# KevynUtopia/Frequency-Aware-Inverse-Consistent-OCTA-Super-Resolution

Measured on AMD Instinct MI355X. Metric: train-step images/sec (G+D fwd+bwd) on 256x256 OCTA, higher is better.
Workload: dtype f32 (tensors and accumulators fp32; the convolutions' operands enter the matrix cores as f16x2 pairs: hi = f16(x 2^k), lo = f16(x 2^k - hi), k from the tensor's largest magnitude; 3 v_mfma_f32_32x32x16_f16 per product) on every map >= 24 wide with >= 16 channels; narrow maps, 1-channel stems / head

## Files before the change

### frequency-aware-inverse-consistent-octa-super-resolution_amd/csrc/common.h

```cpp
#pragma once
#include <hip/hip_runtime.h>
#include <cstdio>
#include <cstdarg>
#include "faoctasr.h"

namespace faoctasr {

char* err_buf();
int fail(int code, const char* fmt, ...);
enum Route { ROUTE_NONE = 0, ROUTE_GATHER_FLAT = 1, ROUTE_PATCH = 2, ROUTE_WINOGRAD = 3, ROUTE_BF16X3 = 4, ROUTE_M1_FWD = 5, ROUTE_NARROW = 6,
             ROUTE_WGRAD_FLAT = 11, ROUTE_WGRAD_PATCH = 12, ROUTE_WGRAD_S1 = 13, ROUTE_M1_WGRAD = 14, ROUTE_WGRAD_X3 = 15, ROUTE_STEM_DGRAD = 7, ROUTE_STEM_WGRAD = 16,
             ROUTE_NARROW_X2 = 8 };
void set_route(int r);
extern thread_local int g_no_split_k;
extern thread_local unsigned* g_out_absmax;
unsigned* take_out_absmax();

void lds_optin(const void* kernel, size_t lds_bytes);

inline int check_launch(const char* what) {
    hipError_t e = hipGetLastError();
    if (e != hipSuccess) return fail(FAOCTASR_EHIP, "%s: %s", what, hipGetErrorString(e));
    return FAOCTASR_OK;
}

__device__ __forceinline__ float act_apply(float v, int act, float slope) {
    switch (act) {
        case FAOCTASR_ACT_RELU: return v > 0.f ? v : 0.f;
        case FAOCTASR_ACT_LRELU: return v > 0.f ? v : v * slope;
        case FAOCTASR_ACT_TANH: return tanhf(v);
        default: return v;
    }
}
__device__ __forceinline__ float act_grad_from_out(float y, int act, float slope) {
    switch (act) {
        case FAOCTASR_ACT_RELU: return y > 0.f ? 1.f : 0.f;
        case FAOCTASR_ACT_LRELU: return y > 0.f ? 1.f : slope;
        case FAOCTASR_ACT_TANH: return 1.f - y * y;
        default: return 1.f;
    }
}

template <class T>
__device__ __forceinline__ T wave_sum(T v) {
#pragma unroll
    for (int o = 32; o > 0; o >>= 1) v += __shfl_xor(v, o, 64);
    return v;
}

template <class T>
__device__ __forceinline__ T block_sum_256(T v, T* red ) {
    v = wave_sum(v);
    __syncthreads();
    if ((threadIdx.x & 63) == 0) red[threadIdx.x >> 6] = v;
    __syncthreads();
    return red[0] + red[1] + red[2] + red[3];
}

__device__ __forceinline__ void block_partial_store_256(float v, float* red , float* part) {
    v = block_sum_256(v, red);
    if (threadIdx.x == 0) part[blockIdx.x] = v;
}

template <class T>
__device__ __forceinline__ double strided_sum_256(const T* __restrict__ p, long n) {
    double a = 0.0;
    for (long i = threadIdx.x; i < n; i += 256) a += (double)p[i];
    return a;
}

__device__ __forceinline__ double block_tree_256(double v, double* red ) {
    red[threadIdx.x] = v;
    __syncthreads();
    for (int o = 128; o > 0; o >>= 1) {
        if ((int)threadIdx.x < o) red[threadIdx.x] += red[threadIdx.x + o];
        __syncthreads();
    }
    const double s = red[0];
    __syncthreads();
    return s;
}

struct PlaneTile { int plane, y0, x0; };
template <int TY, int TX>
__device__ __forceinline__ PlaneTile plane_tile(int tiles_h, int tiles_w) {
    unsigned bi = blockIdx.x;
    PlaneTile t;
    t.x0 = (int)(bi % (unsigned)tiles_w) * TX; bi /= (unsigned)tiles_w;
    t.y0 = (int)(bi % (unsigned)tiles_h) * TY;
    t.plane = (int)(bi / (unsigned)tiles_h);
    return t;
}

inline bool plane_tiles(long planes, int h, int w, int TY, int TX, int* tiles_h, int* tiles_w, long* blocks) {
    *tiles_h = (h + TY - 1) / TY;
    *tiles_w = (w + TX - 1) / TX;
    const long per_plane = (long)*tiles_h * *tiles_w;
    if (planes > 0x7fffffffL / per_plane) return false;
    *blocks = planes * per_plane;
    return true;
}

}
```

### frequency-aware-inverse-consistent-octa-super-resolution_amd/csrc/conv_m1.hip

```cpp
#include "common.h"

namespace faoctasr {

constexpr int M1_TH = 8, M1_TW = 32, M1_KC = 16;

__global__ __launch_bounds__(256) void conv_m1_fwd_kernel(const float* __restrict__ x, const float* __restrict__ w,
                                                          const float* __restrict__ bias, float* __restrict__ y, int N, int C,
                                                          int H, int W, int KH, int KW, int pad, int act, float slope) {
    extern __shared__ __attribute__((aligned(16))) char smem[];
    float* P = reinterpret_cast<float*>(smem);
    const int PH = M1_TH + KH - 1, PW = M1_TW + KW - 1, PHW = PH * PW, T = KH * KW;
    float* Wl = P + M1_KC * PHW;
    const int tid = threadIdx.x;
    const int tiles_x = (W + M1_TW - 1) / M1_TW, tiles_y = (H + M1_TH - 1) / M1_TH;
    const int n = blockIdx.x / (tiles_x * tiles_y);
    const int r = blockIdx.x - n * tiles_x * tiles_y;
    const int y0 = (r / tiles_x) * M1_TH, x0 = (r % tiles_x) * M1_TW;
    const int ty = tid >> 5, tx = tid & 31;
    const long hw = (long)H * W;
    const float* xn = x + (long)n * C * hw;
    constexpr unsigned OOB = 0x7fffffffu;
    const float invPHW = 1.0f / (float)PHW, invPW = 1.0f / (float)PW;
    float acc = 0.f;
    for (int c0 = 0; c0 < C; c0 += M1_KC) {
        const long bytes = (long)(C - c0) * hw * 4;
        const auto srd = __builtin_amdgcn_make_buffer_rsrc(const_cast<float*>(xn + (long)c0 * hw), 0,
                                                           (int)(bytes < 0x7ffffff0L ? bytes : 0x7ffffff0L), 0x00020000);
        __syncthreads();
        for (int e = tid; e < M1_KC * PHW; e += 256) {
            const int c = (int)(((float)e + 0.5f) * invPHW);
            const int q = e - c * PHW;
            const int py = (int)(((float)q + 0.5f) * invPW);
            const int iy = y0 - pad + py, ix = x0 - pad + (q - py * PW);
            const bool ok = (unsigned)iy < (unsigned)H && (unsigned)ix < (unsigned)W;
            P[e] = __builtin_bit_cast(float, __builtin_amdgcn_raw_buffer_load_b32(srd, ok ? 4u * (unsigned)(c * (int)hw + iy * W + ix) : OOB, 0, 0));
        }
        for (int e = tid; e < M1_KC * T; e += 256) Wl[e] = (c0 + e / T < C) ? w[(long)c0 * T + e] : 0.f;
        __syncthreads();
        const float* pp = P + ty * PW + tx;
        for (int c = 0; c < M1_KC; ++c)
            for (int kh = 0; kh < KH; ++kh)
                for (int kw = 0; kw < KW; ++kw) acc += Wl[c * T + kh * KW + kw] * pp[c * PHW + kh * PW + kw];
    }
    const int oy = y0 + ty, ox = x0 + tx;
    if (oy < H && ox < W) {
        if (bias) acc += bias[0];
        y[(long)n * hw + (long)oy * W + ox] = act_apply(acc, act, slope);
    }
}

__global__ __launch_bounds__(256) void conv_m1_wgrad_kernel(const float* __restrict__ x, const float* __restrict__ dy,
                                                            float* __restrict__ dw, int N, int C, int H, int W, int KH, int KW, int pad,
                                                            int tiles_per_block, int CCH) {
    extern __shared__ __attribute__((aligned(16))) char smem[];
    const int PH = M1_TH + KH - 1, PW = M1_TW + KW - 1, PHW = PH * PW, T = KH * KW;
    float* P = reinterpret_cast<float*>(smem);
    float* D = P + CCH * PHW;
    const int tid = threadIdx.x;
    const int c0 = blockIdx.y * CCH;
    const int cl = tid / T, t = tid - cl * T;
    const bool mine = cl < CCH && c0 + cl < C;
    const int kh = t / KW, kw = t - kh * KW;
    const int tiles_x = (W + M1_TW - 1) / M1_TW, tiles_y = (H + M1_TH - 1) / M1_TH;
    const long ntiles = (long)N * tiles_x * tiles_y;
    const long hw = (long)H * W;
    constexpr unsigned OOB = 0x7fffffffu;
    const float invPHW = 1.0f / (float)PHW, invPW = 1.0f / (float)PW;
    float acc = 0.f;
    long tile = (long)blockIdx.x * tiles_per_block;
    long tend = tile + tiles_per_block;
    tend = tend < ntiles ? tend : ntiles;
    for (; tile < tend; ++tile) {
        const int n = (int)(tile / (tiles_x * tiles_y));
        const int r = (int)(tile - (long)n * tiles_x * tiles_y);
        const int y0 = (r / tiles_x) * M1_TH, x0 = (r % tiles_x) * M1_TW;
        const long bytes = (long)(C - c0) * hw * 4;
        const auto srd = __builtin_amdgcn_make_buffer_rsrc(const_cast<float*>(x + ((long)n * C + c0) * hw), 0,
                                                           (int)(bytes < 0x7ffffff0L ? bytes : 0x7ffffff0L), 0x00020000);
        __syncthreads();
        for (int e = tid; e < CCH * PHW; e += 256) {
            const int c = (int)(((float)e + 0.5f) * invPHW);
            const int q = e - c * PHW;
            const int py = (int)(((float)q + 0.5f) * invPW);
            const int iy = y0 - pad + py, ix = x0 - pad + (q - py * PW);
            const bool ok = (unsigned)iy < (unsigned)H && (unsigned)ix < (unsigned)W;
            P[e] = __builtin_bit_cast(float, __builtin_amdgcn_raw_buffer_load_b32(srd, ok ? 4u * (unsigned)(c * (int)hw + iy * W + ix) : OOB, 0, 0));
        }
        {
            const int py = tid >> 5, px = tid & 31;
            const int oy = y0 + py, ox = x0 + px;
            D[tid] = (oy < H && ox < W) ? dy[(long)n * hw + (long)oy * W + ox] : 0.f;
        }
        __syncthreads();
        if (mine) {
            const float* pp = P + cl * PHW + kh * PW + kw;
#pragma unroll 4
            for (int py = 0; py < M1_TH; ++py)
#pragma unroll 8
                for (int px = 0; px < M1_TW; ++px) acc += D[py * M1_TW + px] * pp[py * PW + px];
        }
    }
    if (mine) atomicAdd(dw + (long)(c0 + cl) * T + t, acc);
}

typedef float m1f4 __attribute__((ext_vector_type(4)));

__device__ __forceinline__ void m1_row6(const float* __restrict__ row, int xq, int W, bool rowok, float (&v)[6]) {
    m1f4 c = {0.f, 0.f, 0.f, 0.f};
    float l = 0.f, r = 0.f;
    if (rowok) {
        c = *reinterpret_cast<const m1f4*>(row + xq);
        if (xq > 0) l = row[xq - 1];
        if (xq + 4 < W) r = row[xq + 4];
    }
    v[0] = l; v[1] = c[0]; v[2] = c[1]; v[3] = c[2]; v[4] = c[3]; v[5] = r;
}

__global__ __launch_bounds__(256) void conv_m1_fwd3_kernel(const float* __restrict__ x, const float* __restrict__ w, const float* __restrict__ bias,
                                                           float* __restrict__ y, int N, int C, int H, int W, int act, float slope) {
    const int wq = W >> 2;
    const long item = (long)blockIdx.x * 256 + threadIdx.x;
    const long total = (long)N * H * wq;
    if (item >= total) return;
    const int xq = (int)(item % wq) * 4;
    const long t = item / wq;
    const int oy = (int)(t % H), n = (int)(t / H);
    const long hw = (long)H * W;
    const float* xn = x + (long)n * C * hw;
    float acc[4] = {0.f, 0.f, 0.f, 0.f};
    for (int c = 0; c < C; ++c) {
        const float* wc = w + c * 9;
        const float* xc = xn + (long)c * hw;
#pragma unroll
        for (int kh = 0; kh < 3; ++kh) {
            const int iy = oy - 1 + kh;
            float v[6];
            m1_row6(xc + (long)iy * W, xq, W, (unsigned)iy < (unsigned)H, v);
#pragma unroll
            for (int kw = 0; kw < 3; ++kw) {
                const float wv = wc[kh * 3 + kw];
#pragma unroll
                for (int p = 0; p < 4; ++p) acc[p] += wv * v[p + kw];
            }
        }
    }
    const float b = bias ? bias[0] : 0.f;
    m1f4 o = {act_apply(acc[0] + b, act, slope), act_apply(acc[1] + b, act, slope), act_apply(acc[2] + b, act, slope), act_apply(acc[3] + b, act, slope)};
    *reinterpret_cast<m1f4*>(y + (long)n * hw + (long)oy * W + xq) = o;
}

constexpr int M1W_CH = 4, M1W_ROWS = 32;
__global__ __launch_bounds__(256) void conv_m1_wgrad3_kernel(const float* __restrict__ x, const float* __restrict__ dy, float* __restrict__ dw, int N,
                                                             int C, int H, int W) {
    const int lane = threadIdx.x & 63, wave = threadIdx.x >> 6;
    const int cgroups = (C + M1W_CH - 1) / M1W_CH, rsegs = (H + M1W_ROWS - 1) / M1W_ROWS;
    const long item = (long)blockIdx.x * 4 + wave;
    if (item >= (long)N * rsegs * cgroups) return;
    const int cg = (int)(item % cgroups);
    const long t = item / cgroups;
    const int rs = (int)(t % rsegs), n = (int)(t / rsegs);
    const int c0 = cg * M1W_CH, r0 = rs * M1W_ROWS, r1 = r0 + M1W_ROWS < H ? r0 + M1W_ROWS : H;
    const long hw = (long)H * W;
    const float* dyn = dy + (long)n * hw;
    float acc[M1W_CH][9];
#pragma unroll
    for (int c = 0; c < M1W_CH; ++c)
#pragma unroll
        for (int k = 0; k < 9; ++k) acc[c][k] = 0.f;
    for (int xq = lane * 4; xq < W; xq += 256) {
        float ring[M1W_CH][3][6];
#pragma unroll
        for (int c = 0; c < M1W_CH; ++c) {
            const bool cok = c0 + c < C;
            const float* xc = x + ((long)n * C + (cok ? c0 + c : 0)) * hw;
            m1_row6(xc + (long)(r0 - 1) * W, xq, W, cok && r0 - 1 >= 0, ring[c][0]);
            m1_row6(xc + (long)r0 * W, xq, W, cok, ring[c][1]);
        }
        for (int oy = r0; oy < r1; ++oy) {
            const m1f4 g = *reinterpret_cast<const m1f4*>(dyn + (long)oy * W + xq);
#pragma unroll
            for (int c = 0; c < M1W_CH; ++c) {
                const bool cok = c0 + c < C;
                const float* xc = x + ((long)n * C + (cok ? c0 + c : 0)) * hw;
                m1_row6(xc + (long)(oy + 1) * W, xq, W, cok && oy + 1 < H, ring[c][2]);
#pragma unroll
                for (int kh = 0; kh < 3; ++kh)
#pragma unroll
                    for (int kw = 0; kw < 3; ++kw)
#pragma unroll
                        for (int p = 0; p < 4; ++p) acc[c][kh * 3 + kw] += g[p] * ring[c][kh][p + kw];
#pragma unroll
                for (int q = 0; q < 6; ++q) { ring[c][0][q] = ring[c][1][q]; ring[c][1][q] = ring[c][2][q]; }
            }
        }
    }
#pragma unroll
    for (int c = 0; c < M1W_CH; ++c)
#pragma unroll
        for (int k = 0; k < 9; ++k) {
            const float s = wave_sum(acc[c][k]);
            if (lane == c * 9 + k && c0 + c < C) atomicAdd(dw + (long)(c0 + c) * 9 + k, s);
        }
}

int launch_conv_m1_fwd(const float* x, const float* w, const float* bias, float* y, int N, int C, int H, int W, int KH, int KW, int pad,
                       int act, float slope, hipStream_t stream) {
    if (KH == 3 && KW == 3 && pad == 1 && (W & 3) == 0 && N > 0 && H > 0) {
        const long total = (long)N * H * (W >> 2);
        hipLaunchKernelGGL(conv_m1_fwd3_kernel, dim3((unsigned)((total + 255) / 256)), dim3(256), 0, stream, x, w, bias, y, N, C, H, W, act, slope);
        return check_launch("conv_m1_fwd3");
    }
    const int PH = M1_TH + KH - 1, PW = M1_TW + KW - 1;
    const size_t lds = ((size_t)M1_KC * PH * PW + (size_t)M1_KC * KH * KW) * 4;
    const long blocks = (long)N * ((W + M1_TW - 1) / M1_TW) * ((H + M1_TH - 1) / M1_TH);
    if (blocks <= 0) return FAOCTASR_OK;
    hipLaunchKernelGGL(conv_m1_fwd_kernel, dim3((unsigned)blocks), dim3(256), lds, stream, x, w, bias, y, N, C, H, W, KH, KW, pad,
                       act, slope);
    return check_launch("conv_m1_fwd");
}

int launch_conv_m1_wgrad(const float* x, const float* dy, float* dw, int N, int C, int H, int W, int KH, int KW, int pad, int accumulate,
                         hipStream_t st) {
    const int T = KH * KW;
    if (!accumulate && hipMemsetAsync(dw, 0, sizeof(float) * (size_t)C * T, st) != hipSuccess) return fail(FAOCTASR_EHIP, "memset dw failed");
    if (KH == 3 && KW == 3 && pad == 1 && (W & 3) == 0 && N > 0 && H > 0) {
        const long items = (long)N * ((H + M1W_ROWS - 1) / M1W_ROWS) * ((C + M1W_CH - 1) / M1W_CH);
        hipLaunchKernelGGL(conv_m1_wgrad3_kernel, dim3((unsigned)((items + 3) / 4)), dim3(256), 0, st, x, dy, dw, N, C, H, W);
        return check_launch("conv_m1_wgrad3");
    }
    const int CCH = 256 / T;
    const int PH = M1_TH + KH - 1, PW = M1_TW + KW - 1;
    const size_t lds = ((size_t)CCH * PH * PW + M1_TH * M1_TW) * 4;
    const int gy = (C + CCH - 1) / CCH;
    const long ntiles = (long)N * ((W + M1_TW - 1) / M1_TW) * ((H + M1_TH - 1) / M1_TH);
    if (ntiles <= 0) return FAOCTASR_OK;
    long gx = 1024 / gy;
    if (gx < 1) gx = 1;
    if (gx > ntiles) gx = ntiles;
    const int tpb = (int)((ntiles + gx - 1) / gx);
    gx = (ntiles + tpb - 1) / tpb;
    auto k = conv_m1_wgrad_kernel;
    lds_optin((const void*)k, lds);
    hipLaunchKernelGGL(k, dim3((unsigned)gx, gy), dim3(256), lds, st, x, dy, dw, N, C, H, W, KH, KW, pad, tpb, CCH);
    return check_launch("conv_m1_wgrad");
}

}
```

### frequency-aware-inverse-consistent-octa-super-resolution_amd/csrc/conv_stem.hip

```cpp
#include "common.h"

namespace faoctasr {

constexpr int ST_TH = 8, ST_TW = 32;

template <int CTRL, int ROW_MASK>
__device__ __forceinline__ float dpp_add(float v) {
    const int t = __builtin_amdgcn_update_dpp(0, __float_as_int(v), CTRL, ROW_MASK, 0xf, true);
    return v + __int_as_float(t);
}
__device__ __forceinline__ float wave_sum_to_lane63(float v) {
    v = dpp_add<0x111, 0xf>(v);
    v = dpp_add<0x112, 0xf>(v);
    v = dpp_add<0x114, 0xf>(v);
    v = dpp_add<0x118, 0xf>(v);
    v = dpp_add<0x142, 0xa>(v);
    v = dpp_add<0x143, 0xc>(v);
    return v;
}

template <int C>
__global__ __launch_bounds__(256) void stem_dgrad_kernel(const float* __restrict__ dy, const float* __restrict__ w, float* __restrict__ dx, int N,
                                                         int M, int OH, int OW) {
    extern __shared__ __attribute__((aligned(16))) char smem[];
    float* Wl = reinterpret_cast<float*>(smem);
    const int tid = threadIdx.x;
    for (int i = tid; i < M * C * 16; i += 256) Wl[i] = w[i];
    __syncthreads();
    const int tiles_x = (OW + ST_TW - 1) / ST_TW, tiles_y = (OH + ST_TH - 1) / ST_TH;
    const int n = blockIdx.x / (tiles_x * tiles_y);
    const int r = blockIdx.x - n * tiles_x * tiles_y;
    const int a = (r / tiles_x) * ST_TH + (tid >> 5), b = (r % tiles_x) * ST_TW + (tid & 31);
    if (a >= OH || b >= OW) return;
    const long ohw = (long)OH * OW;
    const float* dyn = dy + (long)n * M * ohw;
    const bool ru = a > 0, rd = a + 1 < OH, cl = b > 0, cr = b + 1 < OW;
    const long o11 = (long)a * OW + b;
    float acc[C][4];
#pragma unroll
    for (int c = 0; c < C; ++c)
#pragma unroll
        for (int q = 0; q < 4; ++q) acc[c][q] = 0.f;
#pragma unroll 4
    for (int m = 0; m < M; ++m) {
        const float* p = dyn + (long)m * ohw + o11;
        const float d11 = p[0];
        const float d10 = cl ? p[-1] : 0.f, d12 = cr ? p[1] : 0.f;
        const float d01 = ru ? p[-OW] : 0.f, d21 = rd ? p[OW] : 0.f;
        const float d00 = (ru && cl) ? p[-OW - 1] : 0.f, d02 = (ru && cr) ? p[-OW + 1] : 0.f;
        const float d20 = (rd && cl) ? p[OW - 1] : 0.f, d22 = (rd && cr) ? p[OW + 1] : 0.f;
#pragma unroll
        for (int c = 0; c < C; ++c) {
            const float* k = Wl + (m * C + c) * 16;
            acc[c][0] += d11 * k[5] + d10 * k[7] + d01 * k[13] + d00 * k[15];
            acc[c][1] += d12 * k[4] + d11 * k[6] + d02 * k[12] + d01 * k[14];
            acc[c][2] += d21 * k[1] + d20 * k[3] + d11 * k[9] + d10 * k[11];
            acc[c][3] += d22 * k[0] + d21 * k[2] + d12 * k[8] + d11 * k[10];
        }
    }
    const int IW = 2 * OW;
    const long ihw = 4 * ohw;
#pragma unroll
    for (int c = 0; c < C; ++c) {
        float* q = dx + ((long)n * C + c) * ihw + (long)(2 * a) * IW + 2 * b;
        *reinterpret_cast<float2*>(q) = make_float2(acc[c][0], acc[c][1]);
        *reinterpret_cast<float2*>(q + IW) = make_float2(acc[c][2], acc[c][3]);
    }
}

template <int C, int MG>
__global__ __launch_bounds__(256) void stem_wgrad_kernel(const float* __restrict__ x, const float* __restrict__ dy, float* __restrict__ dw, int N,
                                                         int M, int OH, int OW, int tiles_per_block) {
    __shared__ float red[4][MG * C * 16];
    const int tid = threadIdx.x, lane = tid & 63, wave = tid >> 6;
    const int tiles_x = (OW + ST_TW - 1) / ST_TW, tiles_y = (OH + ST_TH - 1) / ST_TH;
    const int ntiles = N * tiles_x * tiles_y;
    const int m0 = blockIdx.y * MG;
    const int IH = 2 * OH, IW = 2 * OW;
    const long ohw = (long)OH * OW, ihw = (long)IH * IW;
    float acc[MG][C][16];
#pragma unroll
    for (int j = 0; j < MG; ++j)
#pragma unroll
        for (int c = 0; c < C; ++c)
#pragma unroll
            for (int t = 0; t < 16; ++t) acc[j][c][t] = 0.f;
    int t1 = (blockIdx.x + 1) * tiles_per_block;
    t1 = t1 < ntiles ? t1 : ntiles;
    for (int tile = blockIdx.x * tiles_per_block; tile < t1; ++tile) {
        const int n = tile / (tiles_x * tiles_y);
        const int r = tile - n * tiles_x * tiles_y;
        const int oy = (r / tiles_x) * ST_TH + (tid >> 5), ox = (r % tiles_x) * ST_TW + (tid & 31);
        if (oy >= OH || ox >= OW) continue;
        float g[MG];
#pragma unroll
        for (int j = 0; j < MG; ++j) g[j] = m0 + j < M ? dy[((long)n * M + m0 + j) * ohw + (long)oy * OW + ox] : 0.f;
        const int iy0 = 2 * oy - 1, ix0 = 2 * ox - 1;
        const bool rt = iy0 >= 0, rb = iy0 + 3 < IH, cl = ix0 >= 0, cr = ix0 + 3 < IW;
#pragma unroll
        for (int c = 0; c < C; ++c) {
            const float* p = x + ((long)n * C + c) * ihw + (long)iy0 * IW + ix0;
            float xp[16];
#pragma unroll
            for (int kh = 0; kh < 4; ++kh) {
                const bool rok = (kh > 0 || rt) && (kh < 3 || rb);
                const float2 mid = rok ? *reinterpret_cast<const float2*>(p + kh * IW + 1) : make_float2(0.f, 0.f);
                xp[kh * 4 + 0] = (rok && cl) ? p[kh * IW] : 0.f;
                xp[kh * 4 + 1] = mid.x;
                xp[kh * 4 + 2] = mid.y;
                xp[kh * 4 + 3] = (rok && cr) ? p[kh * IW + 3] : 0.f;
            }
#pragma unroll
            for (int j = 0; j < MG; ++j)
#pragma unroll
                for (int t = 0; t < 16; ++t) acc[j][c][t] += g[j] * xp[t];
        }
    }
#pragma unroll
    for (int j = 0; j < MG; ++j)
#pragma unroll
        for (int c = 0; c < C; ++c)
#pragma unroll
            for (int t = 0; t < 16; ++t) {
                const float v = wave_sum_to_lane63(acc[j][c][t]);
                if (lane == 63) red[wave][(j * C + c) * 16 + t] = v;
            }
    __syncthreads();
    for (int i = tid; i < MG * C * 16; i += 256) {
        const int j = i / (C * 16), ct = i - j * C * 16;
        if (m0 + j < M) atomicAdd(dw + (long)(m0 + j) * C * 16 + ct, red[0][i] + red[1][i] + red[2][i] + red[3][i]);
    }
}

static bool stem_shape(int C, int IH, int IW, int KH, int KW, int stride, int pad, int reflect) {
    return C >= 1 && C <= 4 && KH == 4 && KW == 4 && stride == 2 && pad == 1 && !reflect && (IH & 1) == 0 && (IW & 1) == 0 && IH >= 4 && IW >= 4;
}

bool stem_wgrad_eligible(int C, int IH, int IW, int KH, int KW, int stride, int pad, int reflect) {
    return stem_shape(C, IH, IW, KH, KW, stride, pad, reflect);
}

bool stem_dgrad_eligible(int C, int IH, int IW, int M, int KH, int KW, int stride, int pad) {
    return stem_shape(C, IH, IW, KH, KW, stride, pad, 0) && (long)M * C * 64 <= 48 * 1024;
}

int launch_stem_dgrad(const float* dy, const float* w, float* dx, int N, int C, int IH, int IW, int M, int KH, int KW, int stride, int pad,
                      hipStream_t s) {
    if (!stem_dgrad_eligible(C, IH, IW, M, KH, KW, stride, pad)) return 0;
    const int OH = IH / 2, OW = IW / 2;
    const long blocks = (long)N * ((OW + ST_TW - 1) / ST_TW) * ((OH + ST_TH - 1) / ST_TH);
    if (blocks <= 0) return 1;
    if (blocks > 0x7fffffffL) return 0;
    const size_t lds = (size_t)M * C * 64;
    auto go = [&](auto k) { hipLaunchKernelGGL(k, dim3((unsigned)blocks), dim3(256), lds, s, dy, w, dx, N, M, OH, OW); };
    if (C == 1) go(stem_dgrad_kernel<1>);
    else if (C == 2) go(stem_dgrad_kernel<2>);
    else if (C == 3) go(stem_dgrad_kernel<3>);
    else go(stem_dgrad_kernel<4>);
    const int rc = check_launch("stem_dgrad");
    return rc == FAOCTASR_OK ? 1 : rc;
}

int launch_stem_wgrad(const float* x, const float* dy, float* dw, int N, int C, int IH, int IW, int M, int KH, int KW, int stride, int pad,
                      int reflect, int accumulate, hipStream_t s) {
    if (!stem_shape(C, IH, IW, KH, KW, stride, pad, reflect)) return 0;
    const int OH = IH / 2, OW = IW / 2;
    const long ntiles = (long)N * ((OW + ST_TW - 1) / ST_TW) * ((OH + ST_TH - 1) / ST_TH);
    if (ntiles > 0x7fffffffL) return 0;
    if (!accumulate && hipMemsetAsync(dw, 0, sizeof(float) * (size_t)M * C * 16, s) != hipSuccess) return fail(FAOCTASR_EHIP, "memset dw failed");
    if (ntiles <= 0) return 1;
    const int MG = C == 1 ? 8 : C == 2 ? 4 : 2;
    const int gy = (M + MG - 1) / MG;
    long slabs = 1024 / gy;
    slabs = slabs < 1 ? 1 : slabs;
    slabs = slabs > ntiles ? ntiles : slabs;
    const int tpb = (int)((ntiles + slabs - 1) / slabs);
    const dim3 grid((unsigned)((ntiles + tpb - 1) / tpb), (unsigned)gy);
    auto go = [&](auto k) { hipLaunchKernelGGL(k, grid, dim3(256), 0, s, x, dy, dw, N, M, OH, OW, tpb); };
    if (C == 1) go(stem_wgrad_kernel<1, 8>);
    else if (C == 2) go(stem_wgrad_kernel<2, 4>);
    else if (C == 3) go(stem_wgrad_kernel<3, 2>);
    else go(stem_wgrad_kernel<4, 2>);
    const int rc = check_launch("stem_wgrad");
    return rc == FAOCTASR_OK ? 1 : rc;
}

}
```

### frequency-aware-inverse-consistent-octa-super-resolution_amd/csrc/pointwise.hip

```cpp
#include <mutex>
#include <unordered_map>
#include "common.h"
#include "split16.h"

namespace faoctasr {

thread_local char g_err[512] = "";
char* err_buf() { return g_err; }
int get_route();
int fail(int code, const char* fmt, ...) {
    va_list ap;
    va_start(ap, fmt);
    vsnprintf(g_err, sizeof(g_err), fmt, ap);
    va_end(ap);
    return code;
}

thread_local int g_route = 0;
thread_local unsigned* g_out_absmax = nullptr;
unsigned* take_out_absmax() {
    unsigned* p = g_out_absmax;
    g_out_absmax = nullptr;
    return p;
}
thread_local int g_no_split_k = 0;
void set_route(int r) { g_route = r; }
int get_route() { return g_route; }

void lds_optin(const void* kernel, size_t lds_bytes) {
    if (lds_bytes <= 64 * 1024) return;
    static std::mutex mu;
    static std::unordered_map<const void*, size_t> granted;
    std::lock_guard<std::mutex> lock(mu);
    size_t& have = granted[kernel];
    if (have >= lds_bytes) return;
    (void)hipFuncSetAttribute(kernel, hipFuncAttributeMaxDynamicSharedMemorySize, (int)lds_bytes);
    have = lds_bytes;
}

static inline int grid_for(long n, int per_block, int cap = 4096) {
    long b = (n + per_block - 1) / per_block;
    if (b < 1) b = 1;
    if (b > cap) b = cap;
    return (int)b;
}

__global__ void bn_eval_fwd_kernel(const float* __restrict__ x, const float* __restrict__ gamma, const float* __restrict__ beta,
                                   const float* __restrict__ rmean, const float* __restrict__ rvar, float* __restrict__ y, int C, int HW,
                                   long total, float eps, int act, float slope) {
    const long stride = (long)gridDim.x * blockDim.x;
    for (long i = (long)blockIdx.x * blockDim.x + threadIdx.x; i < total; i += stride) {
        const int c = (int)((i / HW) % C);
        const float sc = (gamma ? gamma[c] : 1.f) / sqrtf(rvar[c] + eps);
        y[i] = act_apply((x[i] - rmean[c]) * sc + (beta ? beta[c] : 0.f), act, slope);
    }
}

__global__ void bn_eval_bwd_kernel(const float* __restrict__ dy, const float* __restrict__ y, const float* __restrict__ gamma,
                                   const float* __restrict__ rvar, float* __restrict__ dx, int C, int HW, long total, float eps, int act,
                                   float slope) {
    const long stride = (long)gridDim.x * blockDim.x;
    for (long i = (long)blockIdx.x * blockDim.x + threadIdx.x; i < total; i += stride) {
        const int c = (int)((i / HW) % C);
        float g = dy[i];
        if (act != FAOCTASR_ACT_NONE) g *= act_grad_from_out(y[i], act, slope);
        dx[i] = g * (gamma ? gamma[c] : 1.f) / sqrtf(rvar[c] + eps);
    }
}

__global__ void act_fwd_kernel(const float* __restrict__ x, float* __restrict__ y, long n, int act, float slope) {
    const long stride = (long)gridDim.x * blockDim.x;
    const long n4 = n >> 2;
    for (long i = (long)blockIdx.x * blockDim.x + threadIdx.x; i < n4; i += stride) {
        float4 v = reinterpret_cast<const float4*>(x)[i];
        v.x = act_apply(v.x, act, slope); v.y = act_apply(v.y, act, slope);
        v.z = act_apply(v.z, act, slope); v.w = act_apply(v.w, act, slope);
        reinterpret_cast<float4*>(y)[i] = v;
    }
    for (long i = (n4 << 2) + (long)blockIdx.x * blockDim.x + threadIdx.x; i < n; i += stride) y[i] = act_apply(x[i], act, slope);
}

__global__ void act_bwd_kernel(const float* __restrict__ dy, const float* __restrict__ y, float* __restrict__ dx, long n, int act,
                               float slope) {
    const long stride = (long)gridDim.x * blockDim.x;
    const long n4 = n >> 2;
    for (long i = (long)blockIdx.x * blockDim.x + threadIdx.x; i < n4; i += stride) {
        float4 g = reinterpret_cast<const float4*>(dy)[i];
        const float4 v = reinterpret_cast<const float4*>(y)[i];
        g.x *= act_grad_from_out(v.x, act, slope); g.y *= act_grad_from_out(v.y, act, slope);
        g.z *= act_grad_from_out(v.z, act, slope); g.w *= act_grad_from_out(v.w, act, slope);
        reinterpret_cast<float4*>(dx)[i] = g;
    }
    for (long i = (n4 << 2) + (long)blockIdx.x * blockDim.x + threadIdx.x; i < n; i += stride)
        dx[i] = dy[i] * act_grad_from_out(y[i], act, slope);
}

__global__ __launch_bounds__(256) void cat2_act_fwd_kernel(const float* __restrict__ a, const float* __restrict__ b, float* __restrict__ y, int N, long la,
                                    long lb, int act, float slope, unsigned* __restrict__ amax) {
    const long tot = (long)N * (la + lb);
    const long stride = (long)gridDim.x * blockDim.x;
    float mx = 0.f;
    for (long i = (long)blockIdx.x * blockDim.x + threadIdx.x; i < tot; i += stride) {
        const long n = i / (la + lb);
        const long r = i - n * (la + lb);
        const float v = r < la ? a[n * la + r] : b[n * lb + (r - la)];
        const float o = act_apply(v, act, slope);
        y[i] = o;
        mx = fmaxf(mx, fabsf(o));
    }
    if (amax) {
        __shared__ unsigned red[4];
        absmax_publish_block(__builtin_bit_cast(unsigned, mx), amax, red);
    }
}

__global__ void cat2_act_bwd_kernel(const float* __restrict__ dy, const float* __restrict__ y, float* __restrict__ da,
                                    float* __restrict__ db, int N, long la, long lb, int act, float slope) {
    const long tot = (long)N * (la + lb);
    const long stride = (long)gridDim.x * blockDim.x;
    for (long i = (long)blockIdx.x * blockDim.x + threadIdx.x; i < tot; i += stride) {
        const long n = i / (la + lb);
        const long r = i - n * (la + lb);
        float g = dy[i];
        if (act != FAOCTASR_ACT_NONE) g *= act_grad_from_out(y[i], act, slope);
        if (r < la) {
            if (da) da[n * la + r] = g;
        } else if (db) {
            db[n * lb + (r - la)] = g;
        }
    }
}

__global__ void axpby_kernel(const float* __restrict__ a, const float* __restrict__ b, float* __restrict__ y, long n, float alpha,
                             float beta) {
    const long stride = (long)gridDim.x * blockDim.x;
    for (long i = (long)blockIdx.x * blockDim.x + threadIdx.x; i < n; i += stride) y[i] = alpha * a[i] + beta * b[i];
}

__global__ void fill_kernel(float* __restrict__ p, long n, float v) {
    const long stride = (long)gridDim.x * blockDim.x;
    for (long i = (long)blockIdx.x * blockDim.x + threadIdx.x; i < n; i += stride) p[i] = v;
}

__global__ __launch_bounds__(256) void channel_sum_kernel(const float* __restrict__ dy, float* __restrict__ db, int N, int C, int HW,
                                                          long per) {
    __shared__ float red[4];
    const int c = blockIdx.y;
    const long L = (long)N * HW;
    long e0 = (long)blockIdx.x * per, e1 = e0 + per;
    e1 = e1 < L ? e1 : L;
    float s = 0.f;
    if ((HW & 3) == 0) {
        for (long e = e0 + 4L * threadIdx.x; e < e1; e += 1024) {
            const long n = e / HW;
            const float4 v = *reinterpret_cast<const float4*>(dy + ((long)n * C + c) * HW + (e - n * HW));
            s += v.x + v.y + v.z + v.w;
        }
    } else {
        for (long e = e0 + threadIdx.x; e < e1; e += 256) {
            const long n = e / HW;
            s += dy[((long)n * C + c) * HW + (e - n * HW)];
        }
    }
    s = block_sum_256(s, red);
    if (threadIdx.x == 0) atomicAdd(db + c, s);
}

__global__ void reflect_pad_bwd_kernel(const float* __restrict__ dxp, float* __restrict__ dx, long NC, int H, int W, int p) {
    const long tot = NC * H * W;
    const int HP = H + 2 * p, WP = W + 2 * p;
    const long stride = (long)gridDim.x * blockDim.x;
    for (long i = (long)blockIdx.x * blockDim.x + threadIdx.x; i < tot; i += stride) {
        const long nc = i / ((long)H * W);
        const int r = (int)(i - nc * H * W);
        const int yy = r / W, xx = r - yy * W;
        int ry[3], rx[3], ny = 0, nx = 0;
        ry[ny++] = yy + p;
        if (yy >= 1 && yy <= p) ry[ny++] = p - yy;
        if (yy <= H - 2 && yy >= H - 1 - p) ry[ny++] = 2 * (H - 1) - yy + p;
        rx[nx++] = xx + p;
        if (xx >= 1 && xx <= p) rx[nx++] = p - xx;
        if (xx <= W - 2 && xx >= W - 1 - p) rx[nx++] = 2 * (W - 1) - xx + p;
        float s = 0.f;
        for (int a = 0; a < ny; ++a)
            for (int b = 0; b < nx; ++b) s += dxp[(nc * HP + ry[a]) * WP + rx[b]];
        dx[i] = s;
    }
}

__global__ void haar_fwd_kernel(const float* __restrict__ x, float* __restrict__ ll, float* __restrict__ hi, long NC, int H, int W) {
    const int h = H >> 1, w = W >> 1;
    const long tot = NC * h * w;
    const long stride = (long)gridDim.x * blockDim.x;
    for (long i = (long)blockIdx.x * blockDim.x + threadIdx.x; i < tot; i += stride) {
        const long nc = i / ((long)h * w);
        const int r = (int)(i - nc * h * w);
        const int yy = r / w, xx = r - yy * w;
        const float* p = x + (nc * H + 2 * yy) * W + 2 * xx;
        const float2 t = *reinterpret_cast<const float2*>(p);
        const float2 u = *reinterpret_cast<const float2*>(p + W);
        const float a = t.x, b = t.y, c = u.x, d = u.y;
        if (ll) ll[i] = (a + b + c + d) * 0.5f;
        if (hi) {
            float* q = hi + (nc * 3) * h * w + r;
            q[0] = (a + b - c - d) * 0.5f;
            q[(long)h * w] = (a - b + c - d) * 0.5f;
            q[2L * h * w] = (a - b - c + d) * 0.5f;
        }
    }
}

__global__ void haar_inv_kernel(const float* __restrict__ ll, const float* __restrict__ hi, float* __restrict__ x, long NC, int H, int W) {
    const int h = H >> 1, w = W >> 1;
    const long tot = NC * h * w;
    const long stride = (long)gridDim.x * blockDim.x;
    for (long i = (long)blockIdx.x * blockDim.x + threadIdx.x; i < tot; i += stride) {
        const long nc = i / ((long)h * w);
        const int r = (int)(i - nc * h * w);
        const int yy = r / w, xx = r - yy * w;
        const float l = ll ? ll[i] : 0.f;
        float lh = 0.f, hl = 0.f, hh = 0.f;
        if (hi) {
            const float* q = hi + (nc * 3) * h * w + r;
            lh = q[0]; hl = q[(long)h * w]; hh = q[2L * h * w];
        }
        float* p = x + (nc * H + 2 * yy) * W + 2 * xx;
        *reinterpret_cast<float2*>(p) = make_float2((l + lh + hl + hh) * 0.5f, (l + lh - hl - hh) * 0.5f);
        *reinterpret_cast<float2*>(p + W) = make_float2((l - lh + hl - hh) * 0.5f, (l - lh - hl + hh) * 0.5f);
    }
}

__global__ void haar_dfront_fwd_kernel(const float* __restrict__ x, float* __restrict__ y, int N, int H, int W, int mode) {
    const int h = H >> 1, w = W >> 1;
    const long tot = (long)N * h * w;
    const long stride = (long)gridDim.x * blockDim.x;
    for (long i = (long)blockIdx.x * blockDim.x + threadIdx.x; i < tot; i += stride) {
        const long n = i / ((long)h * w);
        const int r = (int)(i - n * h * w);
        const int yy = r / w, xx = r - yy * w;
        const float* p = x + (n * H + 2 * yy) * W + 2 * xx;
        const float2 t = *reinterpret_cast<const float2*>(p);
        const float2 u = *reinterpret_cast<const float2*>(p + W);
        const float a = t.x, b = t.y, c = u.x, d = u.y;
        if (mode == 0) {
            y[i] = (a + b + c + d) * 0.5f;
        } else {
            float* q = y + n * 3 * h * w + r;
            q[0] = (a + b - c - d) * 0.25f + 0.5f;
            q[(long)h * w] = (a - b + c - d) * 0.25f + 0.5f;
            q[2L * h * w] = (a - b - c + d) * 0.25f + 0.5f;
        }
    }
}

__global__ void haar_dfront_bwd_kernel(const float* __restrict__ dy, float* __restrict__ dx, int N, int H, int W, int mode) {
    const int h = H >> 1, w = W >> 1;
    const long tot = (long)N * h * w;
    const long stride = (long)gridDim.x * blockDim.x;
    for (long i = (long)blockIdx.x * blockDim.x + threadIdx.x; i < tot; i += stride) {
        const long n = i / ((long)h * w);
        const int r = (int)(i - n * h * w);
        const int yy = r / w, xx = r - yy * w;
        float l = 0.f, lh = 0.f, hl = 0.f, hh = 0.f;
        if (mode == 0) {
            l = dy[i];
        } else {
            const float* q = dy + n * 3 * h * w + r;
            lh = q[0] * 0.5f; hl = q[(long)h * w] * 0.5f; hh = q[2L * h * w] * 0.5f;
        }
        float* p = dx + (n * H + 2 * yy) * W + 2 * xx;
        *reinterpret_cast<float2*>(p) = make_float2((l + lh + hl + hh) * 0.5f, (l + lh - hl - hh) * 0.5f);
        *reinterpret_cast<float2*>(p + W) = make_float2((l - lh + hl - hh) * 0.5f, (l - lh - hl + hh) * 0.5f);
    }
}

__global__ void freq_mix_fwd_kernel(const float* __restrict__ x, const float* __restrict__ lo_hp, const float* __restrict__ lo_lp,
                                    float* __restrict__ hf, float* __restrict__ lf, long n) {
    const long stride = (long)gridDim.x * blockDim.x;
    for (long i = (long)blockIdx.x * blockDim.x + threadIdx.x; i < n; i += stride) {
        const float xv = x[i];
        hf[i] = (fabsf(xv - lo_hp[i]) + xv) * 0.5f;
        lf[i] = -fabsf(lo_lp[i]);
    }
}

__device__ __forceinline__ float sgn(float v) { return v > 0.f ? 1.f : (v < 0.f ? -1.f : 0.f); }

__global__ void freq_mix_bwd_kernel(const float* __restrict__ x, const float* __restrict__ lo_hp, const float* __restrict__ lo_lp,
                                    const float* __restrict__ g_hf, const float* __restrict__ g_lf, float* __restrict__ s_hp,
                                    float* __restrict__ s_lp, float* __restrict__ dx_direct, long n) {
    const long stride = (long)gridDim.x * blockDim.x;
    for (long i = (long)blockIdx.x * blockDim.x + threadIdx.x; i < n; i += stride) {
        const float gh = g_hf ? g_hf[i] : 0.f, gl = g_lf ? g_lf[i] : 0.f;
        const float sh = 0.5f * gh * sgn(x[i] - lo_hp[i]);
        s_hp[i] = sh;
        s_lp[i] = -gl * sgn(lo_lp[i]);
        dx_direct[i] = 0.5f * gh + sh;
    }
}

__device__ __forceinline__ float loss_term(float a, float b, int kind) {
    if (kind == 0) { const float d = a - b; return d * d; }
    if (kind == 1) return fabsf(a - b);
    return fmaxf(a, 0.f) - a * b + log1pf(expf(-fabsf(a)));
}

__global__ __launch_bounds__(256) void loss_partial_kernel(const float* __restrict__ a, const float* __restrict__ b,
                                                           float* __restrict__ part, long n, int kind) {
    __shared__ float red[4];
    const long stride = (long)gridDim.x * blockDim.x;
    float s = 0.f;
    for (long i = (long)blockIdx.x * blockDim.x + threadIdx.x; i < n; i += stride) s += loss_term(a[i], b[i], kind);
    s = block_sum_256(s, red);
    if (threadIdx.x == 0) part[blockIdx.x] = s;
}

__global__ __launch_bounds__(256) void loss_final_kernel(const float* __restrict__ part, int np, float* __restrict__ out, float scale) {
    __shared__ float red[4];
    float s = 0.f;
    for (int i = threadIdx.x; i < np; i += 256) s += part[i];
    s = block_sum_256(s, red);
    if (threadIdx.x == 0) out[0] = s * scale;
}

__global__ void loss_bwd_kernel(const float* __restrict__ a, const float* __restrict__ b, const float* __restrict__ g,
                                float* __restrict__ d, long n, int kind, float scale, int wrt) {
    const float gs = g[0] * scale;
    const long stride = (long)gridDim.x * blockDim.x;
    for (long i = (long)blockIdx.x * blockDim.x + threadIdx.x; i < n; i += stride) {
        const float av = a[i], bv = b[i];
        float v;
        if (kind == 0) v = 2.f * (av - bv) * (wrt == 0 ? 1.f : -1.f);
        else if (kind == 1) v = sgn(av - bv) * (wrt == 0 ? 1.f : -1.f);
        else v = wrt == 0 ? (1.f / (1.f + expf(-av)) - bv) : -av;
        d[i] = gs * v;
    }
}

__global__ __launch_bounds__(256) void mean_mix_fwd_kernel(const float* __restrict__ a, const float* __restrict__ b,
// ... 378 lines not shown
```

Measured before the change: 139.2.

## Rework M=1 3x3 forward conv with row strips, wave channel split and DPP halos

```diff
diff --git a/frequency-aware-inverse-consistent-octa-super-resolution_amd/csrc/common.h b/frequency-aware-inverse-consistent-octa-super-resolution_amd/csrc/common.h
--- a/frequency-aware-inverse-consistent-octa-super-resolution_amd/csrc/common.h
+++ b/frequency-aware-inverse-consistent-octa-super-resolution_amd/csrc/common.h
@@ -45,6 +45,21 @@
 __device__ __forceinline__ T wave_sum(T v) {
 #pragma unroll
     for (int o = 32; o > 0; o >>= 1) v += __shfl_xor(v, o, 64);
+    return v;
+}
+
+template <int CTRL, int ROW_MASK>
+__device__ __forceinline__ float dpp_add(float v) {
+    const int t = __builtin_amdgcn_update_dpp(0, __float_as_int(v), CTRL, ROW_MASK, 0xf, true);
+    return v + __int_as_float(t);
+}
+__device__ __forceinline__ float wave_sum_to_lane63(float v) {
+    v = dpp_add<0x111, 0xf>(v);
+    v = dpp_add<0x112, 0xf>(v);
+    v = dpp_add<0x114, 0xf>(v);
+    v = dpp_add<0x118, 0xf>(v);
+    v = dpp_add<0x142, 0xa>(v);
+    v = dpp_add<0x143, 0xc>(v);
     return v;
 }
 
diff --git a/frequency-aware-inverse-consistent-octa-super-resolution_amd/csrc/conv_m1.hip b/frequency-aware-inverse-consistent-octa-super-resolution_amd/csrc/conv_m1.hip
--- a/frequency-aware-inverse-consistent-octa-super-resolution_amd/csrc/conv_m1.hip
+++ b/frequency-aware-inverse-consistent-octa-super-resolution_amd/csrc/conv_m1.hip
@@ -105,7 +105,101 @@
 
 typedef float m1f4 __attribute__((ext_vector_type(4)));
 
-__device__ __forceinline__ void m1_row6(const float* __restrict__ row, int xq, int W, bool rowok, float (&v)[6]) {
+__device__ __forceinline__ float m1_from_lower_lane(float v) {
+    return __int_as_float(__builtin_amdgcn_update_dpp(0, __float_as_int(v), 0x138, 0xf, 0xf, true));
+}
+__device__ __forceinline__ float m1_from_upper_lane(float v) {
+    return __int_as_float(__builtin_amdgcn_update_dpp(0, __float_as_int(v), 0x130, 0xf, 0xf, true));
+}
+
+__device__ __forceinline__ m1f4 m1_ld4(const float* __restrict__ row, int xqc) {
+    return *reinterpret_cast<const m1f4*>(reinterpret_cast<const char*>(row) + 4u * (unsigned)xqc);
+}
+
+template <bool WIDE>
+__device__ __forceinline__ void m1_row6(m1f4 c, const float* __restrict__ row, int xq, int W, bool rowok, int lane, float (&v)[6]) {
+    float l = m1_from_lower_lane(c[3]), r = m1_from_upper_lane(c[0]);
+    if (WIDE) {
+        if (lane == 0 && rowok && xq > 0 && xq < W) l = row[xq - 1];
+        if (lane == 63 && rowok && xq + 4 < W) r = row[xq + 4];
+    }
+    v[0] = l; v[1] = c[0]; v[2] = c[1]; v[3] = c[2]; v[4] = c[3]; v[5] = r;
+}
+
+constexpr int M1F_ROWS = 4, M1F_WAVES = 8, M1F_CB = 2;
+template <bool WIDE>
+__global__ __launch_bounds__(64 * M1F_WAVES) void conv_m1_fwd3_kernel(const float* __restrict__ x, const float* __restrict__ w,
+                                                                      const float* __restrict__ bias, float* __restrict__ y, int N, int C, int H,
+                                                                      int W, int act, float slope) {
+    __shared__ m1f4 red[M1F_WAVES][M1F_ROWS][64];
+    const int lane = threadIdx.x & 63, wave = __builtin_amdgcn_readfirstlane(threadIdx.x >> 6);
+    const int segs = (W + 255) >> 8, strips = (H + M1F_ROWS - 1) / M1F_ROWS;
+    const int seg = blockIdx.x % segs;
+    const int t = blockIdx.x / segs;
+    const int r0 = (t % strips) * M1F_ROWS, n = t / strips;
+    const int xq = (seg * 64 + lane) * 4;
+    const bool colok = xq < W;
+    const int xqc = colok ? xq : W - 4;
+    const long hw = (long)H * W;
+    const float* xn = x + (long)n * C * hw;
+    const int cpw = (C + M1F_WAVES - 1) / M1F_WAVES;
+    const int cb = wave * cpw, ce = cb + cpw < C ? cb + cpw : C;
+    m1f4 acc[M1F_ROWS];
+#pragma unroll
+    for (int o = 0; o < M1F_ROWS; ++o) acc[o] = m1f4{0.f, 0.f, 0.f, 0.f};
+    for (int c0 = cb; c0 < ce; c0 += M1F_CB) {
+        m1f4 v[M1F_CB][M1F_ROWS + 2];
+#pragma unroll
+        for (int j = 0; j < M1F_CB; ++j) {
+            const float* xc = xn + (long)(c0 + j < ce ? c0 + j : ce - 1) * hw;
+#pragma unroll
+            for (int i = 0; i < M1F_ROWS + 2; ++i) {
+                const int iy = r0 - 1 + i;
+                v[j][i] = m1_ld4(xc + (long)(iy < 0 ? 0 : iy < H ? iy : H - 1) * W, xqc);
+            }
+        }
+#pragma unroll
+        for (int j = 0; j < M1F_CB; ++j) {
+            const bool cok = c0 + j < ce;
+            const int c = cok ? c0 + j : ce - 1;
+            const float* wc = w + (long)c * 9;
+            const float* xc = xn + (long)c * hw;
+#pragma unroll
+            for (int i = 0; i < M1F_ROWS + 2; ++i) {
+                const int iy = r0 - 1 + i;
+                const bool rowok = cok && (unsigned)iy < (unsigned)H;
+                float r6[6];
+                m1_row6<WIDE>(rowok && colok ? v[j][i] : m1f4{0.f, 0.f, 0.f, 0.f}, xc + (long)iy * W, xq, W, rowok, lane, r6);
+#pragma unroll
+                for (int kh = 0; kh < 3; ++kh) {
+                    const int o = i - kh;
+                    if (o < 0 || o >= M1F_ROWS) continue;
+#pragma unroll
+                    for (int kw = 0; kw < 3; ++kw) {
+                        const float wv = wc[kh * 3 + kw];
+#pragma unroll
+                        for (int p = 0; p < 4; ++p) acc[o][p] += wv * r6[p + kw];
+                    }
+                }
+            }
+        }
+    }
+#pragma unroll
+    for (int o = 0; o < M1F_ROWS; ++o) red[wave][o][lane] = acc[o];
+    __syncthreads();
+    if (threadIdx.x >= 64 * M1F_ROWS) return;
+    const int oy = r0 + wave;
+    m1f4 s = red[0][wave][lane];
+#pragma unroll
+    for (int k = 1; k < M1F_WAVES; ++k) s += red[k][wave][lane];
+    if (oy >= H || !colok) return;
+    const float b = bias ? bias[0] : 0.f;
+    const m1f4 o4 = {act_apply(s[0] + b, act, slope), act_apply(s[1] + b, act, slope), act_apply(s[2] + b, act, slope),
+                     act_apply(s[3] + b, act, slope)};
+    *reinterpret_cast<m1f4*>(y + (long)n * hw + (long)oy * W + xq) = o4;
+}
+
+__device__ __forceinline__ void m1_load_row6(const float* __restrict__ row, int xq, int W, bool rowok, float (&v)[6]) {
     m1f4 c = {0.f, 0.f, 0.f, 0.f};
     float l = 0.f, r = 0.f;
     if (rowok) {
@@ -114,39 +208,6 @@
         if (xq + 4 < W) r = row[xq + 4];
     }
     v[0] = l; v[1] = c[0]; v[2] = c[1]; v[3] = c[2]; v[4] = c[3]; v[5] = r;
-}
-
-__global__ __launch_bounds__(256) void conv_m1_fwd3_kernel(const float* __restrict__ x, const float* __restrict__ w, const float* __restrict__ bias,
-                                                           float* __restrict__ y, int N, int C, int H, int W, int act, float slope) {
-    const int wq = W >> 2;
-    const long item = (long)blockIdx.x * 256 + threadIdx.x;
-    const long total = (long)N * H * wq;
-    if (item >= total) return;
-    const int xq = (int)(item % wq) * 4;
-    const long t = item / wq;
-    const int oy = (int)(t % H), n = (int)(t / H);
-    const long hw = (long)H * W;
-    const float* xn = x + (long)n * C * hw;
-    float acc[4] = {0.f, 0.f, 0.f, 0.f};
-    for (int c = 0; c < C; ++c) {
-        const float* wc = w + c * 9;
-        const float* xc = xn + (long)c * hw;
-#pragma unroll
-        for (int kh = 0; kh < 3; ++kh) {
-            const int iy = oy - 1 + kh;
-            float v[6];
-            m1_row6(xc + (long)iy * W, xq, W, (unsigned)iy < (unsigned)H, v);
-#pragma unroll
-            for (int kw = 0; kw < 3; ++kw) {
-                const float wv = wc[kh * 3 + kw];
-#pragma unroll
-                for (int p = 0; p < 4; ++p) acc[p] += wv * v[p + kw];
-            }
-        }
-    }
-    const float b = bias ? bias[0] : 0.f;
-    m1f4 o = {act_apply(acc[0] + b, act, slope), act_apply(acc[1] + b, act, slope), act_apply(acc[2] + b, act, slope), act_apply(acc[3] + b, act, slope)};
-    *reinterpret_cast<m1f4*>(y + (long)n * hw + (long)oy * W + xq) = o;
 }
 
 constexpr int M1W_CH = 4, M1W_ROWS = 32;
@@ -173,8 +234,8 @@
         for (int c = 0; c < M1W_CH; ++c) {
             const bool cok = c0 + c < C;
             const float* xc = x + ((long)n * C + (cok ? c0 + c : 0)) * hw;
-            m1_row6(xc + (long)(r0 - 1) * W, xq, W, cok && r0 - 1 >= 0, ring[c][0]);
-            m1_row6(xc + (long)r0 * W, xq, W, cok, ring[c][1]);
+            m1_load_row6(xc + (long)(r0 - 1) * W, xq, W, cok && r0 - 1 >= 0, ring[c][0]);
+            m1_load_row6(xc + (long)r0 * W, xq, W, cok, ring[c][1]);
         }
         for (int oy = r0; oy < r1; ++oy) {
             const m1f4 g = *reinterpret_cast<const m1f4*>(dyn + (long)oy * W + xq);
@@ -182,7 +243,7 @@
             for (int c = 0; c < M1W_CH; ++c) {
                 const bool cok = c0 + c < C;
                 const float* xc = x + ((long)n * C + (cok ? c0 + c : 0)) * hw;
-                m1_row6(xc + (long)(oy + 1) * W, xq, W, cok && oy + 1 < H, ring[c][2]);
+                m1_load_row6(xc + (long)(oy + 1) * W, xq, W, cok && oy + 1 < H, ring[c][2]);
 #pragma unroll
                 for (int kh = 0; kh < 3; ++kh)
 #pragma unroll
@@ -205,9 +266,9 @@
 
 int launch_conv_m1_fwd(const float* x, const float* w, const float* bias, float* y, int N, int C, int H, int W, int KH, int KW, int pad,
                        int act, float slope, hipStream_t stream) {
-    if (KH == 3 && KW == 3 && pad == 1 && (W & 3) == 0 && N > 0 && H > 0) {
-        const long total = (long)N * H * (W >> 2);
-        hipLaunchKernelGGL(conv_m1_fwd3_kernel, dim3((unsigned)((total + 255) / 256)), dim3(256), 0, stream, x, w, bias, y, N, C, H, W, act, slope);
+    const long blocks3 = (long)N * ((H + M1F_ROWS - 1) / M1F_ROWS) * ((W + 255) >> 8);
+    if (KH == 3 && KW == 3 && pad == 1 && (W & 3) == 0 && N > 0 && H > 0 && W > 0 && C > 0 && blocks3 <= 0x7fffffffL) {
+        hipLaunchKernelGGL(W > 256 ? conv_m1_fwd3_kernel<true> : conv_m1_fwd3_kernel<false>, dim3((unsigned)blocks3), dim3(64 * M1F_WAVES), 0, stream, x, w, bias, y, N, C, H, W, act, slope);
         return check_launch("conv_m1_fwd3");
     }
     const int PH = M1_TH + KH - 1, PW = M1_TW + KW - 1;
diff --git a/frequency-aware-inverse-consistent-octa-super-resolution_amd/csrc/conv_stem.hip b/frequency-aware-inverse-consistent-octa-super-resolution_amd/csrc/conv_stem.hip
--- a/frequency-aware-inverse-consistent-octa-super-resolution_amd/csrc/conv_stem.hip
+++ b/frequency-aware-inverse-consistent-octa-super-resolution_amd/csrc/conv_stem.hip
@@ -3,21 +3,6 @@
 namespace faoctasr {
 
 constexpr int ST_TH = 8, ST_TW = 32;
-
-template <int CTRL, int ROW_MASK>
-__device__ __forceinline__ float dpp_add(float v) {
-    const int t = __builtin_amdgcn_update_dpp(0, __float_as_int(v), CTRL, ROW_MASK, 0xf, true);
-    return v + __int_as_float(t);
-}
-__device__ __forceinline__ float wave_sum_to_lane63(float v) {
-    v = dpp_add<0x111, 0xf>(v);
-    v = dpp_add<0x112, 0xf>(v);
-    v = dpp_add<0x114, 0xf>(v);
-    v = dpp_add<0x118, 0xf>(v);
-    v = dpp_add<0x142, 0xa>(v);
-    v = dpp_add<0x143, 0xc>(v);
-    return v;
-}
 
 template <int C>
 __global__ __launch_bounds__(256) void stem_dgrad_kernel(const float* __restrict__ dy, const float* __restrict__ w, float* __restrict__ dx, int N,
@@ -36,6 +21,7 @@
     const float* dyn = dy + (long)n * M * ohw;
     const bool ru = a > 0, rd = a + 1 < OH, cl = b > 0, cr = b + 1 < OW;
     const long o11 = (long)a * OW + b;
+    const int up = ru ? -OW : 0, dn = rd ? OW : 0, lf = cl ? -1 : 0, rt = cr ? 1 : 0;
     float acc[C][4];
 #pragma unroll
     for (int c = 0; c < C; ++c)
@@ -45,10 +31,12 @@
     for (int m = 0; m < M; ++m) {
         const float* p = dyn + (long)m * ohw + o11;
         const float d11 = p[0];
-        const float d10 = cl ? p[-1] : 0.f, d12 = cr ? p[1] : 0.f;
-        const float d01 = ru ? p[-OW] : 0.f, d21 = rd ? p[OW] : 0.f;
-        const float d00 = (ru && cl) ? p[-OW - 1] : 0.f, d02 = (ru && cr) ? p[-OW + 1] : 0.f;
-        const float d20 = (rd && cl) ? p[OW - 1] : 0.f, d22 = (rd && cr) ? p[OW + 1] : 0.f;
+        const float t10 = p[lf], t12 = p[rt], t01 = p[up], t21 = p[dn];
+        const float t00 = p[up + lf], t02 = p[up + rt], t20 = p[dn + lf], t22 = p[dn + rt];
+        const float d10 = cl ? t10 : 0.f, d12 = cr ? t12 : 0.f;
+        const float d01 = ru ? t01 : 0.f, d21 = rd ? t21 : 0.f;
+        const float d00 = (ru && cl) ? t00 : 0.f, d02 = (ru && cr) ? t02 : 0.f;
+        const float d20 = (rd && cl) ? t20 : 0.f, d22 = (rd && cr) ? t22 : 0.f;
 #pragma unroll
         for (int c = 0; c < C; ++c) {
             const float* k = Wl + (m * C + c) * 16;
diff --git a/frequency-aware-inverse-consistent-octa-super-resolution_amd/csrc/pointwise.hip b/frequency-aware-inverse-consistent-octa-super-resolution_amd/csrc/pointwise.hip
--- a/frequency-aware-inverse-consistent-octa-super-resolution_amd/csrc/pointwise.hip
+++ b/frequency-aware-inverse-consistent-octa-super-resolution_amd/csrc/pointwise.hip
@@ -97,16 +97,43 @@
 
 __global__ __launch_bounds__(256) void cat2_act_fwd_kernel(const float* __restrict__ a, const float* __restrict__ b, float* __restrict__ y, int N, long la,
                                     long lb, int act, float slope, unsigned* __restrict__ amax) {
-    const long tot = (long)N * (la + lb);
-    const long stride = (long)gridDim.x * blockDim.x;
+    const long stride = (long)gridDim.x * blockDim.x, gid = (long)blockIdx.x * blockDim.x + threadIdx.x;
     float mx = 0.f;
-    for (long i = (long)blockIdx.x * blockDim.x + threadIdx.x; i < tot; i += stride) {
-        const long n = i / (la + lb);
-        const long r = i - n * (la + lb);
-        const float v = r < la ? a[n * la + r] : b[n * lb + (r - la)];
-        const float o = act_apply(v, act, slope);
-        y[i] = o;
-        mx = fmaxf(mx, fabsf(o));
+    if ((((unsigned long)la | (unsigned long)lb) & 3) == 0 &&
+        ((reinterpret_cast<unsigned long>(a) | reinterpret_cast<unsigned long>(b) | reinterpret_cast<unsigned long>(y)) & 15) == 0) {
+        const long qa = la >> 2, qb = lb >> 2, qrow = qa + qb, totq = (long)N * qrow;
+        const bool small = totq <= 0x7fffffffL;
+        const float4* a4 = reinterpret_cast<const float4*>(a);
+        const float4* b4 = reinterpret_cast<const float4*>(b);
+        float4* y4 = reinterpret_cast<float4*>(y);
+        for (long q0 = gid; q0 < totq; q0 += 4 * stride) {
+            float4 v[4];
+#pragma unroll
+            for (int j = 0; j < 4; ++j) {
+                const long q = q0 + j * stride < totq ? q0 + j * stride : q0;
+                const long n = small ? (long)((unsigned)q / (unsigned)qrow) : q / qrow;
+                const long r = q - n * qrow;
+                v[j] = *(r < qa ? a4 + n * qa + r : b4 + n * qb + (r - qa));
+            }
+#pragma unroll
+            for (int j = 0; j < 4; ++j) {
+                const long q = q0 + j * stride;
+                if (q >= totq) break;
+                const float4 o = make_float4(act_apply(v[j].x, act, slope), act_apply(v[j].y, act, slope), act_apply(v[j].z, act, slope),
+                                             act_apply(v[j].w, act, slope));
+                y4[q] = o;
+                mx = fmaxf(fmaxf(mx, fmaxf(fabsf(o.x), fabsf(o.y))), fmaxf(fabsf(o.z), fabsf(o.w)));
+            }
+        }
+    } else {
+        const long tot = (long)N * (la + lb);
+        for (long i = gid; i < tot; i += stride) {
+            const long n = i / (la + lb);
+            const long r = i - n * (la + lb);
+            const float o = act_apply(*(r < la ? a + n * la + r : b + n * lb + (r - la)), act, slope);
+            y[i] = o;
+            mx = fmaxf(mx, fabsf(o));
+        }
     }
     if (amax) {
         __shared__ unsigned red[4];
@@ -166,25 +193,49 @@
     if (threadIdx.x == 0) atomicAdd(db + c, s);
 }
 
+typedef float rp_f4u __attribute__((ext_vector_type(4), aligned(4)));
 __global__ void reflect_pad_bwd_kernel(const float* __restrict__ dxp, float* __restrict__ dx, long NC, int H, int W, int p) {
-    const long tot = NC * H * W;
-    const int HP = H + 2 * p, WP = W + 2 * p;
-    const long stride = (long)gridDim.x * blockDim.x;
-    for (long i = (long)blockIdx.x * blockDim.x + threadIdx.x; i < tot; i += stride) {
-        const long nc = i / ((long)H * W);
-        const int r = (int)(i - nc * H * W);
-        const int yy = r / W, xx = r - yy * W;
-        int ry[3], rx[3], ny = 0, nx = 0;
+    const int HP = H + 2 * p, WP = W + 2 * p, cq = (W + 3) >> 2;
+    const long units = NC * H * cq;
+    const bool small = units <= 0x7fffffffL;
+    const bool vst = (W & 3) == 0 && (reinterpret_cast<unsigned long>(dx) & 15) == 0;
+    const long stride = (long)gridDim.x * blockDim.x;
+    for (long u = (long)blockIdx.x * blockDim.x + threadIdx.x; u < units; u += stride) {
+        const long row = small ? (long)((unsigned)u / (unsigned)cq) : u / cq;
+        const long nc = small ? (long)((unsigned)row / (unsigned)H) : row / H;
+        const int x0 = (int)(u - row * cq) * 4, yy = (int)(row - nc * H);
+        int ry[3], ny = 0;
         ry[ny++] = yy + p;
         if (yy >= 1 && yy <= p) ry[ny++] = p - yy;
         if (yy <= H - 2 && yy >= H - 1 - p) ry[ny++] = 2 * (H - 1) - yy + p;
-        rx[nx++] = xx + p;
-        if (xx >= 1 && xx <= p) rx[nx++] = p - xx;
-        if (xx <= W - 2 && xx >= W - 1 - p) rx[nx++] = 2 * (W - 1) - xx + p;
-        float s = 0.f;
-        for (int a = 0; a < ny; ++a)
-            for (int b = 0; b < nx; ++b) s += dxp[(nc * HP + ry[a]) * WP + rx[b]];
-        dx[i] = s;
+        const float* plane = dxp + nc * HP * WP;
+        float* out = dx + row * W + x0;
+        if (x0 > p && x0 + 3 < W - 1 - p) {
+            float s[4] = {0.f, 0.f, 0.f, 0.f};
+            for (int a = 0; a < ny; ++a) {
+                const rp_f4u t = *reinterpret_cast<const rp_f4u*>(plane + (long)ry[a] * WP + x0 + p);
+#pragma unroll
+                for (int i = 0; i < 4; ++i) s[i] += t[i];
+            }
+            if (vst) {
+                *reinterpret_cast<float4*>(out) = make_float4(s[0], s[1], s[2], s[3]);
+            } else {
+#pragma unroll
+                for (int i = 0; i < 4; ++i) out[i] = s[i];
+            }
+            continue;
+        }
+        for (int i = 0; i < 4 && x0 + i < W; ++i) {
+            const int xx = x0 + i;
+            int rx[3], nx = 0;
+            rx[nx++] = xx + p;
+            if (xx >= 1 && xx <= p) rx[nx++] = p - xx;
+            if (xx <= W - 2 && xx >= W - 1 - p) rx[nx++] = 2 * (W - 1) - xx + p;
+            float s = 0.f;
+            for (int a = 0; a < ny; ++a)
+                for (int b = 0; b < nx; ++b) s += plane[(long)ry[a] * WP + rx[b]];
+            out[i] = s;
+        }
     }
 }
 
```

Result: no change. 139.0 (-0.1%).
